# dist1ll/pomcpp

Measured on AMD Instinct MI355X. Metric: env_steps_per_sec, higher is better.
Workload: dtype int32

## Files before the change

### pomcpp_amd/csrc/pom_kernels.h

```cpp
#ifndef POM_KERNELS_H_
#define POM_KERNELS_H_

#include <hip/hip_ext.h>
#include <hip/hip_runtime.h>

#include <climits>
#include <cstdint>

#include "pom_batch.h"
#include "pom_boardgen_body.h"
#include "pom_packed.h"
#include "pom_policy_body.h"
#include "pom_step_body.h"

enum {
    ROW_BOARD = POM_REC_BOARD,
    ROW_BOMBS = POM_REC_BOMBS,
    ROW_FLAMES = POM_REC_FLAMES,
    ROW_BDEST = POM_REC_DWORDS,
    ROW_STACK = POM_REC_DWORDS + 5,
    ROW_CLAIMS = POM_REC_DWORDS + 5,
    LDS_ROWS = POM_REC_DWORDS + 36
};
static_assert(POM_REC_DWORDS % 2 == 0, "the one-lane shapes move the record in groups of 1 or 2 rows");
// ... 737 lines not shown
            const uint8_t* stage_b = reinterpret_cast<const uint8_t*>(stage);
            const int bytes = (int)(left < OBS_CODE_PASS_ENVS ? left : OBS_CODE_PASS_ENVS) * OBS_CODE_ENV_BYTES;
            uint32_t* out_w = reinterpret_cast<uint32_t*>(out_b);
#pragma unroll
            for (int i = 0; i < (OBS_CODE_PASS_ENVS * OBS_CODE_ENV_BYTES / 4 + 63) / 64; i++) {
                const int idx = lane + 64 * i;
                if (idx < (bytes >> 2)) out_w[idx] = stage_w[idx];
            }
            if (lane < (bytes & 3)) out_b[(bytes & ~3) + lane] = stage_b[(bytes & ~3) + lane];
        }
        obs_lds_order();
    }
}

template <int PE>
__device__ __forceinline__ void pom_observe_tile(const ObserveParams& p, const uint32_t* tile, uint4* stage, int64_t tile_id, int lane)
{
    static_assert(PE * POM_Q <= 64 && 16 % PE == 0, "a pass's queue slots are one round of lanes");
    if (p.dtype == POM_OBS_CODES) pom_observe_tile_codes(p, tile, stage, tile_id, lane);
    else
    for (int q = 0; q < 16 / PE; q++) {
        const int64_t e0 = tile_id * 16 + q * PE;
        if (e0 >= p.n) break;
        const int64_t left = p.n - e0;
        const int VECS = (int)(left < PE ? left : PE) * (OBS_ENV_BYTES / 16);
        constexpr int VECS_MAX = PE * OBS_ENV_BYTES / 16;
        pom_observe_stage<false, PE>(tile, stage, q, lane);
        if (p.dtype == POM_OBS_U8 && !p.per_agent) {
            uint4* out = reinterpret_cast<uint4*>(reinterpret_cast<uint8_t*>(p.planes) + e0 * OBS_ENV_BYTES);
#pragma unroll
            for (int i = 0; i < (VECS_MAX + 63) / 64; i++) {
                const int idx = lane + 64 * i;
                if (idx < VECS) out[idx] = stage[idx];
            }
        } else if (p.dtype == POM_OBS_U8) {
            obs_gather_out<uint8_t, PE>(p, reinterpret_cast<const uint32_t*>(stage), e0, lane);
        } else if (p.dtype == POM_OBS_F16) {
            obs_gather_out<_Float16, PE>(p, reinterpret_cast<const uint32_t*>(stage), e0, lane);
        } else {
            obs_gather_out<float, PE>(p, reinterpret_cast<const uint32_t*>(stage), e0, lane);
        }
        obs_lds_order();
    }
    const int ec = lane >> 2, id = lane & 3;
    const int64_t e = tile_id * 16 + ec;
    if (e < p.n && p.agent_attrs) {
        const uint32_t a0 = tile[(POM_REC_AGENTS + 2 * id) * 16 + ec], a1 = tile[(POM_REC_AGENTS + 2 * id + 1) * 16 + ec];
        const int bc = ag_bombcount((int)a0), mx = ag_max_bombs((int)a1);
        int4* o = reinterpret_cast<int4*>(p.agent_attrs + (e * 4 + id) * POM_OBS_AGENT_ATTRS);
        o[0] = make_int4(ag_x((int)a0), ag_y((int)a0), !ag_dead((int)a0), mx - bc);
        o[1] = make_int4(bc, mx, ag_strength((int)a1), ag_kick((int)a0));
    }
    if (lane < 16 && tile_id * 16 + lane < p.n && p.env_attrs) {
        const uint32_t m = pom_rec_meta(tile + lane, 16), st = (pom_rec_meta2(tile + lane, 16) >> 8) & 0xFF;
        const int status = (int)((st & POM_ST_DONE) ? 1 : 0) | (int)((st & POM_ST_DRAW) ? 2 : 0) | (int)((st & POM_ST_TIMEOUT) ? 4 : 0) |
                           (int)((st & POM_ST_RESTARTED) ? 8 : 0);
        reinterpret_cast<int4*>(p.env_attrs)[tile_id * 16 + lane] =
            make_int4((int)tile[POM_REC_TIMESTEP * 16 + lane], pom_sext8(m), status, (int)((st >> POM_ST_WINNER_SHIFT) & 7) - 1);
    }
}

#ifndef POM_QUAD_WAVES
#define POM_QUAD_WAVES 4
#endif
#ifndef POM_WPB
#define POM_WPB 1
#endif
extern "C" __device__ uint64_t pom_dispatch_id(void) __asm("llvm.amdgcn.dispatch.id");
enum { POM_CHAIN_WAIT_LIMIT_US = 2000000 };
#ifndef POM_CHAIN_WORD_STRIDE
#define POM_CHAIN_WORD_STRIDE 16
#endif

struct PomChainVisit {
    int32_t dist = 0;
    unsigned long long done = 0;
#if defined(POM_CHAIN_DIAG)
    long long t0 = 0, t1 = 0, t2 = 0, rt0 = 0;
    int polls = 0;
    uint32_t visit = 0;
#endif
};
__device__ __forceinline__ uint32_t pom_chain_xcd()
{
    uint32_t x;
    asm volatile("s_getreg_b32 %0, hwreg(HW_REG_XCC_ID)" : "=s"(x));
    return x & 0xFu;
}
__device__ __forceinline__ bool pom_chain_enter(unsigned long long* word, uint32_t chain_xcd, uint32_t chain_seq0, uint32_t tape_len, uint64_t wait_limit,
                                                uint32_t* err, int lane, PomChainVisit& v)
{
    const uint32_t xcd = chain_xcd + 1u;
#if defined(POM_CHAIN_DIAG)
    v.t0 = (long long)__builtin_readcyclecounter();
    v.rt0 = (long long)wall_clock64();
#endif
    unsigned long long w = 0;
    if (lane == 0) w = __hip_atomic_fetch_add(word, 1ull << POM_CHAIN_TICKET_SHIFT, __ATOMIC_RELAXED, __HIP_MEMORY_SCOPE_AGENT);
    w = ((unsigned long long)(uint32_t)__builtin_amdgcn_readfirstlane((int)(w >> 32)) << 32) | (uint32_t)__builtin_amdgcn_readfirstlane((int)(uint32_t)w);
    const uint32_t visit = (uint32_t)(w >> POM_CHAIN_TICKET_SHIFT);
    v.dist = (int32_t)pom_chain_visit_distance(visit, chain_seq0);
#if defined(POM_CHAIN_DIAG)
    v.t1 = (long long)__builtin_readcyclecounter();
#endif
    int polls = 0;
    bool timed_out = false;
    if (!((uint32_t)w & POM_CHAIN_POISON) && (int32_t)pom_chain_visit_distance((uint32_t)w & POM_CHAIN_COUNT_MASK, visit) < 0) {
        const uint64_t t_wait0 = wall_clock64();
        for (;;) {
            __builtin_amdgcn_s_sleep(1);
            w = __hip_atomic_load(word, __ATOMIC_RELAXED, __HIP_MEMORY_SCOPE_AGENT);
            w = ((unsigned long long)(uint32_t)__builtin_amdgcn_readfirstlane((int)(w >> 32)) << 32) | (uint32_t)__builtin_amdgcn_readfirstlane((int)(uint32_t)w);
            polls++;
            if (((uint32_t)w & POM_CHAIN_POISON) || (int32_t)pom_chain_visit_distance((uint32_t)w & POM_CHAIN_COUNT_MASK, visit) >= 0) break;
            if (wall_clock64() - t_wait0 >= wait_limit) {
                timed_out = true;
                break;
            }
        }
    }
    (void)polls;
    const uint32_t was_on = (uint32_t)(w >> 32) & 0xFu;
    const bool poisoned = ((uint32_t)w & POM_CHAIN_POISON) != 0;
    const bool wrong_xcd = was_on != 0u && was_on != xcd;
    const bool off_tape = tape_len != 0u && (uint32_t)v.dist >= tape_len;
    if (poisoned || timed_out || wrong_xcd || off_tape) {
        if (lane == 0 && !poisoned) {
            __hip_atomic_fetch_or(word, (unsigned long long)POM_CHAIN_POISON, __ATOMIC_RELAXED, __HIP_MEMORY_SCOPE_AGENT);
            __hip_atomic_fetch_or(err, (uint32_t)(timed_out ? POM_CHAIN_E_TIMEOUT : wrong_xcd ? POM_CHAIN_E_XCD : POM_CHAIN_E_TAPE), __ATOMIC_RELAXED,
                                  __HIP_MEMORY_SCOPE_AGENT);
        }
        return false;
    }
#if defined(POM_CHAIN_DIAG)
    v.t2 = (long long)__builtin_readcyclecounter();
    v.polls = polls;
    v.visit = visit;
#endif
    v.done = 1ull + ((unsigned long long)(xcd - was_on) << 32);
    return true;
}
__device__ __forceinline__ void pom_chain_leave(unsigned long long* word, int lane, const PomChainVisit& v)
{
    asm volatile("s_waitcnt vmcnt(0)" ::: "memory");
    if (lane == 0) __hip_atomic_fetch_add(word, v.done, __ATOMIC_RELAXED, __HIP_MEMORY_SCOPE_AGENT);
}

template <bool CHAIN>
__device__ __forceinline__ uint32_t pom_load_shared(const uint32_t* ptr)
{
    return CHAIN ? __hip_atomic_load(ptr, __ATOMIC_RELAXED, __HIP_MEMORY_SCOPE_AGENT) : *ptr;
}

template <int EPW, int G, bool FRESH, bool POLICY = false, bool ATEND = false, bool SINGLE = false, bool CHAIN = false, bool OBS = false>
__global__ __launch_bounds__(64 * POM_WPB, (POLICY ? 4 : G == 4 ? POM_QUAD_WAVES : EPW == 16 ? 3 : EPW == 32 ? 2 : 1)) void pom_step_kernel(StepParams p)
{
    static_assert(!CHAIN || SINGLE, "chained launches play one tick each");
    static_assert(!OBS || (SINGLE && !CHAIN && !POLICY && POM_WPB == 1), "the fused observation exists for the one-tick explicit-move shape");
    static_assert(!SINGLE || G == 4, "the one-tick instantiation exists for the quad shape");
    static_assert(G == 1 || (G == 4 && EPW == 16), "a quad per env needs 16 envs per wavefront");
    static_assert(!POLICY || G == 4, "the policy runs one agent per lane of the quad");
    static_assert(!ATEND || G == 4, "the end-of-tick reset is built for the quad shape only");
    constexpr int OBS_ROWS = (obs_stage_vecs(OBS_PASS_ENVS_FUSED) * 16 + EPW * 4 - 1) / (EPW * 4);
    constexpr int OVERLAY = POLICY ? 44 : OBS ? OBS_ROWS : 0;
    constexpr int ROWS = POM_REC_DWORDS + OVERLAY > LDS_ROWS ? POM_REC_DWORDS + OVERLAY : LDS_ROWS;
    static_assert(ROWS >= LDS_ROWS, "the tick's scratch rows fit under the overlay");
    __shared__ __attribute__((aligned(16))) uint32_t tiles_[POM_WPB][ROWS * EPW];
    uint32_t* const tile = tiles_[POM_WPB == 1 ? 0 : threadIdx.x >> 6];
    uint8_t* const danger = reinterpret_cast<uint8_t*>(tile + POM_REC_DWORDS * EPW);
    uint32_t* const sets = tile + (POM_REC_DWORDS + 32) * EPW;
    const int lane = threadIdx.x & 63;
    int64_t tile_local;
    uint32_t chain_xcd = 0;
    if (CHAIN) {
        chain_xcd = pom_chain_xcd();
        const int64_t q = gridDim.x / 8;
        int64_t k_in_xcd = (int64_t)(blockIdx.x / 8) + p.chain_rot;
        if (k_in_xcd >= q) k_in_xcd -= q;
        tile_local = (int64_t)chain_xcd * q + k_in_xcd;
        if (chain_xcd >= 8u) {
            if (lane == 0) __hip_atomic_fetch_or(p.chain_err, (uint32_t)POM_CHAIN_E_XCD, __ATOMIC_RELAXED, __HIP_MEMORY_SCOPE_AGENT);
            return;
        }
        if (POM_WPB == 1 && p.block0 + tile_local >= p.block_end) return;
    } else {
#if defined(POM_NO_XCD_REMAP)
    tile_local = blockIdx.x;
#else
    {
        const int64_t b = blockIdx.x, nb = gridDim.x, q = nb / 8, r = nb % 8, x = b % 8;
        tile_local = (x < r ? x * (q + 1) : r * (q + 1) + (x - r) * q) + b / 8;
    }
#endif
    }
    if (POM_WPB > 1) {
        tile_local = tile_local * POM_WPB + (threadIdx.x >> 6);
        if (p.block0 + tile_local >= p.block_end) return;
    }
    const int64_t tile_id = p.block0 + tile_local;
    const int64_t np = p.n_pad;
    const bool env_mode = p.mode == POM_MODE_ENV;
    const int el = lane % EPW, sub = lane / EPW;
    const int64_t e_d = tile_id * EPW + el;
    uint32_t* col_d = p.state + pom_rec_col(e_d);
    const int ec = G == 1 ? el : lane >> 2;
    const int member = G == 1 ? 0 : lane & 3;
    const int64_t e = tile_id * EPW + ec;
    const bool owner = G == 1 ? sub == 0 : member == 0;
    const bool runs = G == 1 ? sub == 0 : true;
    const bool valid = runs && e < p.n;
    const uint32_t env_key = (uint32_t)(p.env_offset + e);
    uint32_t* t = tile + ec;

#if defined(POM_DIAG)
    const long long t_begin = (long long)clock64();
#endif
    long long c_steps = 0, c_episodes = 0, c_resets = 0, c_ub = 0;

    uint32_t tick0 = CHAIN ? p.tick0 : p.tick0 + *p.tick_base;
    PomChainVisit cv;
    if (CHAIN) {
        unsigned long long* const word = p.tile_seq + tile_id * POM_CHAIN_WORD_STRIDE;
        if (!pom_chain_enter(word, chain_xcd, p.chain_seq0, p.tape_len, p.chain_wait_limit, p.chain_err, lane, cv)) return;
        tick0 += (uint32_t)cv.dist;
        load_tile16_x4<POM_REC_DWORDS, 16>(p.state + tile_id * POM_TILE_DWORDS, POM_TILE_ENVS, tile, lane);
    } else if (EPW == 16) load_tile16_x4(p.state + tile_id * POM_TILE_DWORDS, POM_TILE_ENVS, tile, lane);
    else load_tile<EPW>(col_d, POM_TILE_ENVS, tile, sub);
    uint32_t m0 = 0, m1 = 0;
    if (POLICY) {
        m0 = pom_load_shared<CHAIN>(p.agent_mem + tile_id * 64 + lane);
        m1 = pom_load_shared<CHAIN>(p.agent_mem + 4 * np + tile_id * 64 + lane);
    }
    uint64_t draw0 = 0;
    int4 moves0 = make_int4(0, 0, 0, 0);
    constexpr bool TAKES_MOVES = SINGLE || G == 1;
    if (!POLICY) {
        if (TAKES_MOVES && p.moves) {
            if (valid) moves0 = reinterpret_cast<const int4*>(p.moves)[(CHAIN ? (int64_t)cv.dist * p.n : (int64_t)0) + e];
        } else {
            if (G == 4 && !SINGLE) {
            } else if (G == 4) draw0 = pom_rng_draw_half(p.seed, env_key, tick0, member >> 1);
            else draw0 = pom_rng_draw(p.seed, env_key, tick0);
        }
    }
    asm volatile("s_waitcnt vmcnt(0)" ::: "memory");
    PomLane L;
    int time_step = 0;
    uint32_t status = 0;
    lane_from_tile(L, time_step, status, t, EPW);
    bool restarted = false;

    LdsEnv<EPW, G> acc(tile, ec, member);
    PomStepper<LdsEnv<EPW, G>> stepper(acc, L);
#if defined(POM_TRUNC)
    L.trunc = p.trunc;
#endif
#if defined(POM_DIAG)
    for (int k = 0; k < POM_PH_N; k++) L.t_acc[k] = 0;
    L.t_last = t_begin;
    POM_STAMP(L, POM_PH_LOAD);
#endif

    const int n_ticks = SINGLE ? 1 : p.ticks;
    for (int tk = 0; tk < n_ticks; tk++) {
        if (ATEND) {
        } else if (FRESH) {
            const bool reload = valid && env_mode && p.auto_reset == POM_RESET_AT_START && (status & POM_ST_DONE);
            uint64_t todo = __ballot(reload && owner);
            while (todo) {
                const int src = __builtin_amdgcn_readfirstlane(__ffsll((unsigned long long)todo) - 1);
                todo &= todo - 1;
                const int ec_u = G == 1 ? src : src >> 2;
                uint32_t ep = 0;
                if (lane == src) {
                    ep = pom_load_shared<CHAIN>(p.episode + e) + 1u;
                    p.episode[e] = ep;
                }
                ep = (uint32_t)__builtin_amdgcn_readfirstlane(__shfl((int)ep, src));
                const uint32_t key = pom_board_key(p.board_seed, (uint32_t)(p.env_offset + tile_id * EPW + ec_u), ep);
                pom_boardgen_wave<EPW, POM_REC_DWORDS>(tile, ec_u, (uint32_t)__builtin_amdgcn_readfirstlane((int)key), lane);
            }
            asm volatile("" ::: "memory");
            if (reload) lane_from_tile(L, time_step, status, t, EPW);
            restarted = reload;
            c_resets += __popcll(__ballot(reload && owner));
        } else {
            const bool reload = valid && env_mode && p.auto_reset == POM_RESET_AT_START && (status & POM_ST_DONE);
            uint64_t todo = __ballot(reload && owner);
            if (todo) {
                c_resets += __popcll(todo);
                int lane_now = lane;
                if (!SINGLE) asm volatile("" : "+v"(lane_now));
                do {
                    const int src = __builtin_amdgcn_readfirstlane(__ffsll((unsigned long long)todo) - 1);
                    todo &= todo - 1;
                    const int ec_u = G == 1 ? src : src >> 2;
                    restart_column<EPW>(tile, ec_u, p.snap + (tile_id * EPW + ec_u) * POM_REC_DWORDS, lane_now);
                } while (todo);
                asm volatile("" ::: "memory");
                if (reload) lane_from_tile(L, time_step, status, t, EPW);
            }
            restarted = reload;
        }
        const bool active = valid && !(env_mode && (status & POM_ST_DONE));
        bool newly_done = false, new_ub = false;
        int mv_own = POM_MOVE_IDLE;
        if (POLICY) {
            if (tk > 0) {
                m0 = p.agent_mem[tile_id * 64 + lane];
                m1 = p.agent_mem[4 * np + tile_id * 64 + lane];
            }
            if (restarted) m0 = m1 = 0;
            restarted = false;
            PolicyStore st{tile, t, danger + ec, sets + ec, member};
#if defined(POM_TRUNC)
            st.trunc = p.trunc;
            if (active) {
                if (p.trunc > -4) pom_policy_prepare_clear(st);
                if (p.trunc > -3) pom_policy_prepare_fill(st, PomPolicyEnv{{L.a0[0], L.a0[1], L.a0[2], L.a0[3]}, {acc.ag1(0), acc.ag1(1), acc.ag1(2), acc.ag1(3)}, L.bIdx, L.bCnt});
                if (p.trunc > -2) pom_policy_prepare_safe(st);
            }
            if (p.trunc > -1)
#else
            if (active) {
                pom_policy_prepare_clear(st);
                pom_policy_prepare_fill(st, PomPolicyEnv{{L.a0[0], L.a0[1], L.a0[2], L.a0[3]}, {acc.ag1(0), acc.ag1(1), acc.ag1(2), acc.ag1(3)}, L.bIdx, L.bCnt});
                pom_policy_prepare_safe(st);
            }
#endif
            {
                const PomPolicyEnv E{{L.a0[0], L.a0[1], L.a0[2], L.a0[3]}, {acc.ag1(0), acc.ag1(1), acc.ag1(2), acc.ag1(3)}, L.bIdx, L.bCnt};
                const uint32_t r = pom_rng_draw_half(p.seed, env_key, tick0 + (uint32_t)tk, member >> 1);
                const bool actor = active && !ag_dead(sel4(member, L.a0));
#if defined(POM_DIAG)
                long long pt_last = 0, pt_acc[POM_PP_N];
                mv_own = pom_policy_wave(st, E, member, m0, m1, actor, (int)((((r >> (16 * (member & 1))) & 0xFFFFu) * 5u) >> 16), sets, lane, pt_last, pt_acc);
#else
                mv_own = pom_policy_wave(st, E, member, m0, m1, actor, (int)((((r >> (16 * (member & 1))) & 0xFFFFu) * 5u) >> 16), sets, lane);
#endif
            }
            p.agent_mem[tile_id * 64 + lane] = m0;
            p.agent_mem[4 * np + tile_id * 64 + lane] = m1;
        }
        if (active) {
            uint32_t mvp;
            if (G == 4) {
                int mine;
                if (POLICY) {
                    mine = mv_own;
                } else if (TAKES_MOVES && p.moves) {
                    const int lo = (member & 1) ? moves0.y : moves0.x, hi = (member & 1) ? moves0.w : moves0.z;
                    mine = (member & 2) ? hi : lo;
                } else {
                    const uint32_t r = SINGLE ? (uint32_t)draw0 : pom_rng_draw_half(p.seed, env_key, tick0 + (uint32_t)tk, member >> 1);
                    mine = pom_rng_pick((r >> (16 * (member & 1))) & 0xFFFFu, p.dist);
                }
                mvp = stepper.pack_moves_quad(mine);
            } else {
                int mv[4];
                if (p.moves) {
                    mv[0] = moves0.x; mv[1] = moves0.y; mv[2] = moves0.z; mv[3] = moves0.w;
                } else {
                    const uint64_t r = tk == 0 ? draw0 : pom_rng_draw(p.seed, env_key, tick0 + (uint32_t)tk);
#pragma unroll
                    for (int i = 0; i < 4; i++) mv[i] = pom_rng_pick((uint32_t)(r >> (16 * i)) & 0xFFFFu, p.dist);
                }
                mvp = stepper.pack_moves(mv);
            }
            L.ub = 0;
            status &= ~(uint32_t)POM_ST_RESTARTED;
            POM_STAMP(L, POM_PH_RESTART);
#if defined(POM_TRUNC)
            if (p.trunc <= 0) {
            } else
#endif
            if (POLICY) {
                uint32_t* t2 = tile;
                asm volatile("" : "+v"(t2));
                LdsEnv<EPW, G> acc2(t2, ec, member);
                PomStepper<LdsEnv<EPW, G>> stepper2(acc2, L);
                stepper2.step_packed(mvp);
            } else {
                stepper.step_packed(mvp);
            }
            new_ub = L.ub != 0;
            L.ub |= (t[(POM_REC_AGENTS + 5) * EPW] >> 24) | ((t[(POM_REC_AGENTS + 7) * EPW] >> 24) << 8);
            if (env_mode) {
                time_step = (int)t[POM_REC_TIMESTEP * EPW] + 1;
                if (owner) t[POM_REC_TIMESTEP * EPW] = (uint32_t)time_step;
                status = pom_env_epilogue(L, time_step, p.max_steps, status);
                newly_done = (status & POM_ST_DONE) != 0;
            }
        }
        c_steps += __popcll(__ballot(active && owner));
        c_episodes += __popcll(__ballot(newly_done && owner));
        c_ub += __popcll(__ballot(new_ub && owner));
        if (ATEND) {
            uint64_t todo = __ballot(newly_done && owner);
            if (todo) {
                c_resets += __popcll(todo);
                if (newly_done && owner) {
#pragma unroll
                    for (int k = 0; k < 8; k++) t[(POM_REC_AGENTS + k) * EPW] = pom_lane_agent_word(L, status, k, t[(POM_REC_AGENTS + k) * EPW]);
                }
                asm volatile("" ::: "memory");
                int lane_end = lane;
                asm volatile("" : "+v"(lane_end));
                do {
                    const int src = __builtin_amdgcn_readfirstlane(__ffsll((unsigned long long)todo) - 1);
                    todo &= todo - 1;
                    const int ec_u = G == 1 ? src : src >> 2;
                    const int64_t e_u = tile_id * EPW + ec_u;
                    uint32_t* tr = p.terminal + e_u * POM_REC_DWORDS;
                    column_to_record<EPW>(tile, ec_u, tr, lane_end);
                    if (FRESH) {
                        uint32_t ep = 0;
                        if (lane == src) {
                            ep = pom_load_shared<CHAIN>(p.episode + e_u) + 1u;
                            p.episode[e_u] = ep;
                        }
                        ep = (uint32_t)__builtin_amdgcn_readfirstlane(__shfl((int)ep, src));
                        const uint32_t key = pom_board_key(p.board_seed, (uint32_t)(p.env_offset + e_u), ep);
                        pom_boardgen_wave<EPW, POM_REC_DWORDS>(tile, ec_u, (uint32_t)__builtin_amdgcn_readfirstlane((int)key), lane_end);
                    } else {
                        restart_column<EPW>(tile, ec_u, p.snap + e_u * POM_REC_DWORDS, lane_end);
                    }
                } while (todo);
                asm volatile("" ::: "memory");
                if (newly_done && runs) {
                    lane_from_tile(L, time_step, status, t, EPW);
                    status |= POM_ST_RESTARTED;
                    if (POLICY) {
                        int lane_here = lane;
                        asm volatile("" : "+v"(lane_here));
                        p.agent_mem[tile_id * 64 + lane_here] = 0u;
                        p.agent_mem[4 * np + tile_id * 64 + lane_here] = 0u;
                    }
                }
            }
        }
        POM_STAMP(L, POM_PH_EPILOGUE);
    }

    if (owner) {
#pragma unroll
        for (int k = 0; k < 8; k++) t[(POM_REC_AGENTS + k) * EPW] = pom_lane_agent_word(L, status, k, (k & 1) ? t[(POM_REC_AGENTS + k) * EPW] : 0u);
    }
    if (EPW == 16) {
        int lane_late = lane;
        asm volatile("" : "+v"(lane_late));
        store_tile16_x4<CHAIN>(p.state + tile_id * POM_TILE_DWORDS, POM_TILE_ENVS, tile, lane_late);
    } else {
        store_tile<EPW>(col_d, POM_TILE_ENVS, tile, sub, el);
    }
    if (OBS) {
        asm volatile("s_waitcnt lgkmcnt(0)" ::: "memory");
        ObserveParams op;
        op.state = nullptr;
        op.n = p.n;
        op.n_pad = p.n_pad;
        op.block0 = 0;
        op.planes = p.obs_planes;
        op.agent_attrs = p.obs_agent_attrs;
        op.env_attrs = p.obs_env_attrs;
        op.dtype = p.obs_dtype;
        op.per_agent = p.obs_per_agent;
        pom_observe_tile<OBS_PASS_ENVS_FUSED>(op, tile, reinterpret_cast<uint4*>(tile + POM_REC_DWORDS * EPW), tile_id, lane);
    }
    if (CHAIN) {
        pom_chain_leave(p.tile_seq + tile_id * POM_CHAIN_WORD_STRIDE, lane, cv);
#if defined(POM_CHAIN_DIAG)
        if (lane == 0) {
            unsigned long long* d = p.tile_seq + (p.block_end - p.block0) * POM_CHAIN_WORD_STRIDE + 68 * tile_id;
            d[4 + 2 * (cv.visit & 31)] = (unsigned long long)cv.rt0;
            d[5 + 2 * (cv.visit & 31)] = (unsigned long long)wall_clock64();
            d[0] += (unsigned long long)(cv.t1 - cv.t0);
            d[1] += (unsigned long long)(cv.t2 - cv.t1);
            d[2] += (unsigned long long)((long long)__builtin_readcyclecounter() - cv.t0);
            d[3] += (unsigned long long)cv.polls;
        }
#endif
    }

#if defined(POM_DIAG)
    asm volatile("s_waitcnt vmcnt(0)" ::: "memory");
    POM_STAMP(L, POM_PH_STORE);
    if (p.diag) {
        long long inside = 0;
        for (int k = POM_PH_X_SCAN; k <= POM_PH_X_SHORT; k++) inside += L.t_acc[k];
        long long best = inside;
        for (int o = 32; o > 0; o >>= 1) {
            const long long w = __shfl_xor(best, o);
            best = w > best ? w : best;
        }
        const uint64_t who = __ballot(inside == best);
        if (lane == __ffsll((unsigned long long)who) - 1)
            for (int k = 0; k < POM_PH_N; k++) p.diag[tile_id * POM_PH_N + k] += L.t_acc[k];
    }
#endif
    if (lane == 0) {
        unsigned long long* wc = reinterpret_cast<unsigned long long*>(p.wave_counters + tile_id * POM_CNT_N);
        __hip_atomic_fetch_add(&wc[POM_CNT_STEPS], (unsigned long long)c_steps, __ATOMIC_RELAXED, __HIP_MEMORY_SCOPE_AGENT);
        if (c_episodes) __hip_atomic_fetch_add(&wc[POM_CNT_EPISODES], (unsigned long long)c_episodes, __ATOMIC_RELAXED, __HIP_MEMORY_SCOPE_AGENT);
        if (c_resets) __hip_atomic_fetch_add(&wc[POM_CNT_RESETS], (unsigned long long)c_resets, __ATOMIC_RELAXED, __HIP_MEMORY_SCOPE_AGENT);
        if (c_ub) __hip_atomic_fetch_add(&wc[POM_CNT_UB_TICKS], (unsigned long long)c_ub, __ATOMIC_RELAXED, __HIP_MEMORY_SCOPE_AGENT);
    }
}

struct LitmusParams {
    uint32_t* data;
    unsigned long long* tile_seq;
    uint32_t* err;
    unsigned long long* out;
    int64_t tiles;
    uint32_t chain_seq0;
    uint64_t wait_limit;
};
__global__ __launch_bounds__(64) void pom_chain_litmus_kernel(LitmusParams p)
// ... 464 lines not shown
```

### pomcpp_amd/csrc/pom_step_body.h

```cpp
#ifndef POM_STEP_BODY_H_
#define POM_STEP_BODY_H_

#include "pom_packed.h"

#if defined(__clang__)
#define POM_NOUNROLL _Pragma("nounroll")
#else
#define POM_NOUNROLL
#endif
#define POM_N 11
#define POM_Q 20
#define POM_STACK_DEPTH 21

#if defined(POM_DIAG) && defined(__HIP_DEVICE_COMPILE__)
#define POM_STAMP(L, k)                                   \
    do {                                                  \
        const long long now_ = (long long)clock64();      \
        (L).t_acc[k] += now_ - (L).t_last;                \
        (L).t_last = now_;                                \
    } while (0)
#else
#define POM_STAMP(L, k) ((void)0)
#endif
#if defined(POM_TRUNC)
#define POM_CUT(L, k)                 \
    do {                              \
        if ((L).trunc <= (k)) return; \
    } while (0)
#else
#define POM_CUT(L, k) ((void)0)
#endif
enum { POM_PH_LOAD = 0, POM_PH_FLAMES, POM_PH_AGENT_PREP, POM_PH_AGENT_LOOP, POM_PH_BOMB_PASS, POM_PH_BOMB_A, POM_PH_BOMB_B,
       POM_PH_TICK_BOMBS, POM_PH_EPILOGUE, POM_PH_STORE,
       POM_PH_X_SCAN, POM_PH_X_COMMIT, POM_PH_X_EPILOGUE, POM_PH_X_NEST, POM_PH_X_SHORT, POM_PH_RESTART, POM_PH_FLAMES_DEC, POM_PH_N };

struct PomLane {
    int a0[4];
    int alive, bIdx, bCnt, fIdx, fCnt;
    uint32_t ub;
#if defined(POM_DIAG)
    long long t_last, t_acc[POM_PH_N];
#endif
#if defined(POM_TRUNC)
    int trunc;
#endif
};

POM_HD int pc_is_wood(int e) { return (unsigned)(e - POM_C_WOOD) < 5u; }
POM_HD int pc_is_powerup(int e) { return (unsigned)(e - POM_C_EXTRABOMB) < 3u; }
POM_HD int pc_is_walkable(int e) { return (int)pc_is_powerup(e) | (int)(e == 0); }
POM_HD int pc_is_flame(int e) { return e >= POM_C_FLAME; }
POM_HD int pc_is_agent(int e) { return (unsigned)(e - POM_C_AGENT) < 4u; }
POM_HD int pc_agent_id(int e) { return e - POM_C_AGENT; }
POM_HD int pc_wood_flag(int e) { return (e - POM_C_WOOD) & 3; }
POM_HD int pc_is_static_block(int e) { return (int)((unsigned)(e - POM_C_EXTRABOMB) < 8u) | (int)(e == POM_C_RIGID); }
POM_HD int pc_blocks_bomb(int e) { return (int)((unsigned)(e - POM_C_EXTRABOMB) < 12u) | (int)(e == POM_C_RIGID); }
POM_HD int pc_flag_item(int f) { return f == 0 ? 0 : f + (POM_C_EXTRABOMB - 1); }
POM_HD int pc_flame_code(int c0, int r, int i, int f) { return f == 0 ? POM_C_FLAME + c0 : POM_C_FLAGGED - 41 + 40 * f + 10 * r + i; }
POM_HD int pc_flame_pops_to(int e, int c0, int r, int i)
{
    const int k = e - (POM_C_FLAGGED - 1) - 10 * r - i;
    const int flagged = (int)(k == 0) | (int)(k == 40) | (int)(k == 80);
    const int item = POM_C_EXTRABOMB + (int)(k >= 40) + (int)(k >= 80);
    return e == POM_C_FLAME + c0 ? POM_C_PASSAGE : flagged ? item : -1;
}

POM_HD int pb_x(int b) { return b & 0xF; }
POM_HD int pb_y(int b) { return (b >> 4) & 0xF; }
POM_HD int pb_pos(int b) { return b & 0xFF; }
POM_HD int pb_id(int b) { return (b >> 8) & 0xF; }
POM_HD int pb_strength(int b) { return (b >> 12) & 0xF; }
POM_HD int pb_time(int b) { return (b >> 16) & 0xF; }
POM_HD int pb_dir(int b) { return (b >> 20) & 0xF; }
POM_HD int pb_set(int b, uint32_t mask, uint32_t v) { return (int)(((uint32_t)b & ~mask) + v); }

#if defined(__HIP_DEVICE_COMPILE__)
#define POM_IN_VGPR(x) asm("" : "+v"(x))
#else
#define POM_IN_VGPR(x) ((void)0)
#endif
POM_HD int sel4(int i, const int v[4])
{
    int v0 = v[0], v1 = v[1], v2 = v[2], v3 = v[3];
    POM_IN_VGPR(v0);
    POM_IN_VGPR(v1);
    POM_IN_VGPR(v2);
    POM_IN_VGPR(v3);
    const int lo = (i & 1) ? v1 : v0, hi = (i & 1) ? v3 : v2;
    return (i & 2) ? hi : lo;
}
POM_HD uint32_t pick4(int i, const uint32_t v[4])
{
    const uint32_t lo = (i & 1) ? v[1] : v[0], hi = (i & 1) ? v[3] : v[2];
    return (i & 2) ? hi : lo;
}
POM_HD void put4(int i, int v[4], int x)
{
    v[0] = i == 0 ? x : v[0];
    v[1] = i == 1 ? x : v[1];
    v[2] = i == 2 ? x : v[2];
    v[3] = i == 3 ? x : v[3];
}
POM_HD int ag_x(int a0) { return a0 & 0xF; }
POM_HD int ag_y(int a0) { return (a0 >> 4) & 0xF; }
POM_HD int ag_pos(int a0) { return a0 & 0xFF; }
POM_HD int ag_dead(int a0) { return (a0 >> 17) & 1; }
POM_HD int ag_kick(int a0) { return (a0 >> 16) & 1; }
POM_HD int ag_setpos(int a0, int x, int y) { return (a0 & ~0xFF) | x | (y << 4); }
POM_HD int ag_bombcount(int a0) { return pom_sext8((uint32_t)a0 >> 8); }
POM_HD int ag_bombcount_add(int a0, int d) { return (a0 & ~0xFF00) | (int)(((uint32_t)a0 + ((uint32_t)d << 8)) & 0xFF00u); }
POM_HD int ag_max_bombs(int a1) { return pom_sext16((uint32_t)a1); }
POM_HD int ag_strength(int a1) { return (a1 >> 16) & 0xFF; }
POM_HD int ag_strength_inc(int a1) { return ag_strength(a1) == 0xFF ? a1 : a1 + (1 << 16); }

POM_HD int wrap20(int p)
{
    const unsigned u = (unsigned)p, w = u - (unsigned)POM_Q;
    return (int)(u < w ? u : w);
}
POM_HD uint32_t pom_zero_bytes(uint32_t x)
{
    return ~(((x & 0x7F7F7F7Fu) + 0x7F7F7F7Fu) | x | 0x7F7F7F7Fu);
}
POM_HD int div11(int c)
{
#if defined(__HIP_DEVICE_COMPILE__)
    return __mul24(c, 373) >> 12;
#else
    return c / POM_N;
#endif
}
POM_HD int oob(int x, int y)
{
    const unsigned ux = (unsigned)x, uy = (unsigned)y;
    return (ux > uy ? ux : uy) >= (unsigned)POM_N;
}

POM_HD int mv_dx(int m) { return (int)((0x55555615u >> (2 * m)) & 3u) - 1; }
POM_HD int mv_dy(int m) { return (int)((0x55555561u >> (2 * m)) & 3u) - 1; }

template <class A>
struct PomStepper {
    A& a;
    PomLane& L;
    uint32_t oldp_ = 0;
    int irregular_ = 0;
    int folded_ = 0;
    uint32_t occ_[4] = {0u, 0u, 0u, 0u};
    int occ_valid_ = 0, occ_keep_ = 0;
    POM_HD PomStepper(A& a_, PomLane& l_) : a(a_), L(l_) {}

    POM_HD int bomb_at(int i) const { return a.bomb(wrap20(L.bIdx + i)); }
    POM_HD void set_bomb_at(int i, int v) { a.set_bomb(wrap20(L.bIdx + i), v); }

    POM_HD int bomb_index(int pos) const
    {
        int r = 99;
        POM_NOUNROLL
        for (int i = a.sub(); i < L.bCnt; i += A::G) {
            if (pb_pos(bomb_at(i)) == pos) {
                r = i;
                break;
            }
        }
        r = a.gmin(r);
        return r == 99 ? -1 : r;
    }
    POM_HD void put_bomb_at(int i, int v) { a.put_bomb(wrap20(L.bIdx + i), v); }
    POM_HD int bomb_index_alone(int pos) const
    {
        POM_NOUNROLL
        for (int i = 0; i < L.bCnt; i += 4) {
            const int b0 = bomb_at(i), b1 = bomb_at(i + 1), b2 = bomb_at(i + 2), b3 = bomb_at(i + 3);
            int r = -1;
            r = ((int)(i + 3 < L.bCnt) & (int)(pb_pos(b3) == pos)) ? i + 3 : r;
            r = ((int)(i + 2 < L.bCnt) & (int)(pb_pos(b2) == pos)) ? i + 2 : r;
            r = ((int)(i + 1 < L.bCnt) & (int)(pb_pos(b1) == pos)) ? i + 1 : r;
            r = pb_pos(b0) == pos ? i : r;
            if (r >= 0) return r;
        }
        return -1;
    }

    POM_HD int get_agent(int x, int y) const
    {
        const int want = x | (y << 4);
        int r = -1;
#pragma unroll
        for (int i = 3; i >= 0; i--)
            r = ((!ag_dead(L.a0[i])) & (int)(ag_pos(L.a0[i]) == want)) ? i : r;
        return r;
    }

    POM_HD void kill(int id)
    {
        if (id >= POM_AGENT_COUNT) {
            L.ub |= POM_UB_BAD_INDEX;
            return;
        }
        int v = sel4(id, L.a0);
        if (!ag_dead(v)) {
            put4(id, L.a0, v | POM_AG_DEAD);
            L.alive--;
        }
    }

    POM_HD void owner_bombcount_dec(int b)
    {
        int id = pb_id(b);
        if (id >= POM_AGENT_COUNT) {
            L.ub |= POM_UB_BAD_INDEX;
            return;
        }
        put4(id, L.a0, ag_bombcount_add(sel4(id, L.a0), -1));
    }

    POM_HD void remove_at(int at)
    {
        POM_NOUNROLL
        for (int i = at + 1 + a.sub(); i < L.bCnt; i += A::G) {
            const int v = bomb_at(i);
            put_bomb_at(i - 1, v);
        }
        a.sync();
        if (folded_) {
            const int w = bomb_at(L.bCnt - 1);
            set_bomb_at(L.bCnt - 1, (w & (1 << 24)) ? (w & ~(1 << 24)) : (int)((uint32_t)w + (1u << 16)));
        }
        L.bCnt--;
    }

    enum { REM_TOP = 62, REM_NONE = 63 };

    POM_HD int owner_strength(int b)
    {
        const int owner = pb_id(b);
        if (owner < POM_AGENT_COUNT) return ag_strength(a.ag1(owner));
        L.ub |= POM_UB_BAD_INDEX;
        return 0;
    }
// ... 469 lines not shown
                POM_NOUNROLL
                for (int i = a.sub(); i < L.bCnt; i += A::G) {
                    if (a.bdest(i) == okey) {
                        bd = i;
                        break;
                    }
                }
                bd = a.gmin(bd);
                if (bd == 99) bd = -1;
            }
            put4(id, L.a0, ag_setpos(av, ox, oy));
            irregular_ |= (ox | (oy << 4)) != (int)((oldp_ >> (8 * id)) & 0xFF);
            a.set_cell(oy * POM_N + ox, POM_C_AGENT + id);
            if (origin_agent != -1) {
                id = origin_agent;
                continue;
            }
            if (bd != -1) {
                const int b = bomb_at(bd);
                const int dir = pb_dir(b);
                if (mv_dx(dir) == 0 && mv_dy(dir) == 0) {
                    a.set_cell(oy * POM_N + ox, POM_C_AGENT + id);
                    return;
                }
                const int bx = ox - mv_dx(dir), by = oy - mv_dy(dir);
                if (oob(bx, by)) {
                    L.ub |= POM_UB_BAD_INDEX;
                    return;
                }
                const int has_agent = get_agent(bx, by);
                set_bomb_at(bd, pb_set(pb_set(b, 0xF00000u, 0), 0xFFu, (uint32_t)bx + ((uint32_t)by << 4)));
                a.set_cell(by * POM_N + bx, POM_C_BOMB);
                if (has_agent != -1) {
                    id = has_agent;
                    continue;
                }
            }
            return;
        }
    }

    POM_HD int bomb_target_key(int b) const
    {
        const int d = pb_dir(b);
        return (pb_x(b) + mv_dx(d) + 1) | ((pb_y(b) + mv_dy(d) + 1) << 4);
    }

    POM_HD int bomb_collision(uint32_t mvp, int k)
    {
        const int b = bomb_at(k);
        const int key = bomb_target_key(b);
        int collided = 0;
        POM_NOUNROLL
        for (int i = k + a.sub(); i < L.bCnt; i += A::G) {
            const int o = bomb_at(i);
            if (o != b && bomb_target_key(o) == key) {
                put_bomb_at(i, pb_set(o, 0xF00000u, 0));
                collided = 1;
            }
        }
        collided = a.gor(collided);
        if (collided && pb_dir(b) != 0) {
            const int nb = pb_set(b, 0xF00000u, 0);
            set_bomb_at(k, nb);
            const int ag = get_agent(pb_x(nb), pb_y(nb));
            if (ag > -1) {
                const int m = (mvp >> (4 * ag)) & 0xF;
                if (m != POM_MOVE_IDLE && m != POM_MOVE_BOMB) {
                    unforeseen_ = 1;
                    chain_reversion(mvp, ag);
                    const int cur = bomb_at(k);
                    a.set_cell(pb_y(cur) * POM_N + pb_x(cur), POM_C_BOMB);
                }
            }
        }
        return collided;
    }

    POM_HD void loop_a_bomb(int mvp, int oldp, int k, int bombs_move)
    {
        const int b = bomb_at(k);
        const int bx = pb_x(b), by = pb_y(b), d = pb_dir(b);
        const int tx = bx + mv_dx(d), ty = by + mv_dy(d);
        int blocked = oob(tx, ty);
        if (!blocked) {
            const int e = a.cell(ty * POM_N + tx);
            blocked = pc_blocks_bomb(e);
        }
        if (blocked) {
            set_bomb_at(k, pb_set(b, 0xF00000u, 0));
            const int ag = get_agent(bx, by);
            if (ag > -1) {
                const int m = (mvp >> (4 * ag)) & 0xF;
                const int av = sel4(ag, L.a0);
                const int was = (oldp >> (8 * ag)) & 0xFF;
                if ((int)(m != POM_MOVE_IDLE) & (int)(m != POM_MOVE_BOMB) & (int)((ag_x(av) | (ag_y(av) << 4)) != was)) {
                    chain_reversion(mvp, ag, bombs_move);
                    if (get_agent(bx, by) == -1) a.set_cell(by * POM_N + bx, POM_C_BOMB);
                }
            }
        }
    }

    POM_HD void step(const int mv_in[4]) { step_packed(pack_moves(mv_in)); }
    POM_HD static int clamp_move(int m) { return ((unsigned)m <= 5u) ? m : 6; }
    POM_HD static uint32_t pack_moves(const int mv_in[4])
    {
        uint32_t mvp = 0;
#pragma unroll
        for (int i = 0; i < 4; i++) mvp |= (uint32_t)clamp_move(mv_in[i]) << (4 * i);
        return mvp;
    }
    POM_HD uint32_t pack_moves_quad(int mine) const
    {
        const int c = clamp_move(mine);
        return (uint32_t)a.template gbcast<0>(c) | ((uint32_t)a.template gbcast<1>(c) << 4) | ((uint32_t)a.template gbcast<2>(c) << 8) |
               ((uint32_t)a.template gbcast<3>(c) << 12);
    }
    POM_HD void step_packed(uint32_t mvp)
    {
        int ftop, fn, btop, bn;
        flames_dec(ftop, fn);
        POM_STAMP(L, POM_PH_FLAMES_DEC);
        POM_CUT(L, 10);
        flame_pops(ftop, fn);
        POM_STAMP(L, POM_PH_FLAMES);
        POM_CUT(L, 20);
        step_middle(mvp, btop, bn);
        top_explosions(btop, bn);
        POM_STAMP(L, POM_PH_TICK_BOMBS);
    }
    POM_HD void top_explosions(int top, int n)
    {
        occ_valid_ = 0;
        occ_keep_ = 1;
        POM_NOUNROLL
        for (int k = 0; k < n && L.bCnt > 0; k++) {
            const int c = k == 0 ? top : bomb_at(0);
            if (pb_time(c) != 0) break;
            explode(pb_x(c), pb_y(c), pb_strength(c), REM_TOP, c);
        }
        occ_valid_ = occ_keep_ = 0;
    }
    POM_HD void prep_positions(const uint32_t mvp, uint32_t& oldp, uint32_t& dstp, int& deadmask, int& contact, int& clash)
    {
        oldp = dstp = 0;
        deadmask = 0;
#pragma unroll
        for (int i = 0; i < 4; i++) deadmask |= ag_dead(L.a0[i]) << i;
        contact = 0;
        clash = 0;
        if (A::G == 4) {
            const int m = a.sub();
            const int av = sel4(m, L.a0);
            const int mvm = (int)((mvp >> (4 * m)) & 0xF);
            const int pxm = ag_x(av), pym = ag_y(av);
            const int dxm = pxm + mv_dx(mvm), dym = pym + mv_dy(mvm);
            const int pos8 = ag_pos(av);
            oldp = (uint32_t)a.template gbcast<0>(pos8) | ((uint32_t)a.template gbcast<1>(pos8) << 8) |
                   ((uint32_t)a.template gbcast<2>(pos8) << 16) | ((uint32_t)a.template gbcast<3>(pos8) << 24);
            const int d8 = ((dxm + 1) & 0xF) | (((dym + 1) & 0xF) << 4);
            dstp = (uint32_t)a.template gbcast<0>(d8) | ((uint32_t)a.template gbcast<1>(d8) << 8) |
                   ((uint32_t)a.template gbcast<2>(d8) << 16) | ((uint32_t)a.template gbcast<3>(d8) << 24);
            const uint32_t want = (uint32_t)((dxm & 0xF) | ((dym & 0xF) << 4));
            const uint32_t others = ~(0x80u << (8 * m));
            const uint32_t dead80 = (((uint32_t)deadmask * 0x00204081u) & 0x01010101u) << 7;
            const uint32_t hit_d = pom_zero_bytes(oldp ^ (want * 0x01010101u)) & others;
            const uint32_t hit_p = pom_zero_bytes(oldp ^ ((uint32_t)pos8 * 0x01010101u)) & others & ~dead80;
            int mine = (int)(hit_d != 0u) | ((int)((hit_p != 0u) & !ag_dead(av)) << 1);
            mine = a.gor(mine);
            contact = mine & 1;
            clash = mine >> 1;
        } else {
#pragma unroll
            for (int i = 0; i < 4; i++) {
                const int px = ag_x(L.a0[i]), py = ag_y(L.a0[i]);
                const int mvi = (int)((mvp >> (4 * i)) & 0xF);
                const int dx = px + mv_dx(mvi), dy = py + mv_dy(mvi);
                oldp |= (uint32_t)(px | (py << 4)) << (8 * i);
                dstp |= (uint32_t)(((dx + 1) & 0xF) | (((dy + 1) & 0xF) << 4)) << (8 * i);
            }
#pragma unroll
            for (int i = 0; i < 4; i++)
#pragma unroll
                for (int j = 0; j < 4; j++)
                    if (i != j) contact |= ((((dstp >> (8 * i)) & 0xF) - 1) & 0xF) == ((oldp >> (8 * j)) & 0xF) &&
                                           ((((dstp >> (8 * i + 4)) & 0xF) - 1) & 0xF) == ((oldp >> (8 * j + 4)) & 0xF);
        }
    }
    POM_HD void prep_dependencies(const uint32_t mvp, const uint32_t oldp, const int deadmask, uint32_t& dstp, uint32_t& dep, uint32_t& roots,
                                  int& nroots)
    {
        int px[4], py[4], dx[4], dy[4];
#pragma unroll
        for (int i = 0; i < 4; i++) {
            px[i] = (int)((oldp >> (8 * i)) & 0xF);
            py[i] = (int)((oldp >> (8 * i + 4)) & 0xF);
            const int mvi = (int)((mvp >> (4 * i)) & 0xF);
            dx[i] = px[i] + mv_dx(mvi);
            dy[i] = py[i] + mv_dy(mvi);
        }
        roots = 0xFFFF;
        nroots = 0;
#pragma unroll
        for (int i = 0; i < 4; i++) {
#pragma unroll
            for (int j = i; j < 4; j++) {
                if ((int)(dx[i] == px[j]) & (int)(dy[i] == py[j]) & (int)(dx[j] == px[i]) & (int)(dy[j] == py[i])) {
                    dx[i] = px[i]; dy[i] = py[i];
                    dx[j] = px[j]; dy[j] = py[j];
                }
            }
        }
#pragma unroll
        for (int i = 0; i < 4; i++) {
            int is_root = 1;
            if (!((deadmask >> i) & 1)) {
#pragma unroll
                for (int j = 0; j < 4; j++) {
                    if (j == i) continue;
                    if (is_root & !((deadmask >> j) & 1) & (int)(dx[i] == px[j]) & (int)(dy[i] == py[j])) {
                        dep = (dep & ~(0xFu << (4 * j))) | ((uint32_t)i << (4 * j));
                        is_root = 0;
                    }
                }
            }
            if (is_root) {
                roots = (roots & ~(0xFu << (4 * nroots))) | ((uint32_t)i << (4 * nroots));
                nroots++;
            }
        }
        dstp = 0;
#pragma unroll
        for (int i = 0; i < 4; i++) dstp |= (uint32_t)(((dx[i] + 1) & 0xF) | (((dy[i] + 1) & 0xF) << 4)) << (8 * i);
    }

    int unforeseen_ = 0;
    POM_HD uint32_t loop_b_todo()
    {
        a.claims_clear();
        a.sync();
        POM_NOUNROLL
        for (int k = a.sub(); k < L.bCnt; k += A::G) {
            const int b = bomb_at(k);
            const int d = pb_dir(b);
            const int bx = pb_x(b), by = pb_y(b), tx = bx + mv_dx(d), ty = by + mv_dy(d);
            a.claim(by * POM_N + bx);
            if ((int)(d != 0) & !oob(tx, ty) & (int)((mv_dx(d) | mv_dy(d)) != 0)) a.claim(ty * POM_N + tx);
        }
        a.sync();
        uint32_t f = 0;
        POM_NOUNROLL
        for (int k = a.sub(); k < L.bCnt; k += A::G) {
            const int b = bomb_at(k);
            const int c = pb_y(b) * POM_N + pb_x(b);
            const int e = a.cell(c);
            f |= (uint32_t)((int)(pb_dir(b) != 0) | (int)(e == POM_C_PASSAGE) | pc_is_flame(e) | (int)(a.claims(c) >= 2)) << k;
        }
        return (uint32_t)a.gor((int)f);
    }
    POM_HD void loop_b_bomb(uint32_t mvp, int k)
    {
        int b = bomb_at(k);
        const int bx = pb_x(b), by = pb_y(b), d = pb_dir(b);
        int tx = bx, ty = by;
        if (d == 0) {
            if (bomb_collision(mvp, k)) return;
            const int c = by * POM_N + bx;
            const int e = a.cell(c);
            if (e == POM_C_PASSAGE) a.set_cell(c, POM_C_BOMB);
            if (!pc_is_flame(e)) return;
        } else {
            tx = bx + mv_dx(d);
            ty = by + mv_dy(d);
            int free_way = !oob(tx, ty);
            int tc = 0, te = 0;
            if (free_way) {
                tc = ty * POM_N + tx;
                te = a.cell(tc);
                free_way = !pc_is_static_block(te);
            }
            if (!free_way) {
                set_bomb_at(k, pb_set(b, 0xF00000u, 0));
                return;
            }
            if (bomb_collision(mvp, k)) return;
            b = bomb_at(k);
            set_bomb_at(k, pb_set(b, 0xFFu, (uint32_t)tx + ((uint32_t)ty << 4)));
            if (bomb_index(bx | (by << 4)) < 0 && a.cell(by * POM_N + bx) == POM_C_BOMB)
                a.set_cell(by * POM_N + bx, POM_C_PASSAGE);
            te = a.cell(tc);
            if (pc_is_walkable(te)) a.set_cell(tc, POM_C_BOMB);
            if (!pc_is_flame(te)) return;
        }
        const int j = bomb_index(tx | (ty << 4));
        const int jb = bomb_at(j);
        unforeseen_ = 1;
        explode(pb_x(jb), pb_y(jb), owner_strength(jb), j);
    }

    POM_HD void step_middle(const uint32_t mvp, int& top, int& n)
    {
        top = 0;
        n = 0;

        uint32_t oldp = 0, dstp = 0;
        uint32_t dep = 0xFFFF, roots = 0x3210;
        int nroots = 4;
        int deadmask = 0, contact = 0, clash = 0;
        prep_positions(mvp, oldp, dstp, deadmask, contact, clash);
        oldp_ = oldp;
        POM_CUT(L, 24);
        if (contact) prep_dependencies(mvp, oldp, deadmask, dstp, dep, roots, nroots);
        POM_CUT(L, 27);
        const int ouroboros = nroots == 0;
        int posb[4];
#pragma unroll
        for (int i = 0; i < 4; i++) posb[i] = (int)((oldp >> (8 * i)) & 0xFF);

        int on_bomb = 0;
        POM_NOUNROLL
        for (int k = a.sub(); k < L.bCnt; k += A::G) {
// ... 385 lines not shown
```

Measured before the change: 8.936 billion.

## Build quad old positions locally, drop VGPR pins, specialise uniform move pick

In the quad prep path, the packed old-position word is now built directly from the agent records each lane already holds, instead of four cross-lane broadcasts. The own agent's position and dead flag are then taken from that word and the dead mask. The VGPR-pinning asm is removed from sel4. Random move picking goes through a helper that does a plain multiply-shift for the non-stress distributions, with empty asm barriers added around the branches. Together these aim to cut cross-lane traffic and selection overhead, but the asm barriers may also constrain scheduling.

```diff
diff --git a/pomcpp_amd/csrc/pom_kernels.h b/pomcpp_amd/csrc/pom_kernels.h
--- a/pomcpp_amd/csrc/pom_kernels.h
+++ b/pomcpp_amd/csrc/pom_kernels.h
@@ -913,6 +913,19 @@
     return CHAIN ? __hip_atomic_load(ptr, __ATOMIC_RELAXED, __HIP_MEMORY_SCOPE_AGENT) : *ptr;
 }
 
+__device__ __forceinline__ int pom_pick_uniform(uint32_t r16, int dist)
+{
+    int mv;
+    if (dist == POM_DIST_STRESS) {
+        asm volatile("");
+        mv = pom_rng_pick(r16, POM_DIST_STRESS);
+    } else {
+        asm volatile("");
+        mv = (int)((r16 * (dist == POM_DIST_HARMLESS ? 5u : 6u)) >> 16);
+    }
+    return mv;
+}
+
 template <int EPW, int G, bool FRESH, bool POLICY = false, bool ATEND = false, bool SINGLE = false, bool CHAIN = false, bool OBS = false>
 __global__ __launch_bounds__(64 * POM_WPB, (POLICY ? 4 : G == 4 ? POM_QUAD_WAVES : EPW == 16 ? 3 : EPW == 32 ? 2 : 1)) void pom_step_kernel(StepParams p)
 {
@@ -1110,11 +1123,13 @@
                 if (POLICY) {
                     mine = mv_own;
                 } else if (TAKES_MOVES && p.moves) {
+                    asm volatile("");
                     const int lo = (member & 1) ? moves0.y : moves0.x, hi = (member & 1) ? moves0.w : moves0.z;
                     mine = (member & 2) ? hi : lo;
                 } else {
+                    asm volatile("");
                     const uint32_t r = SINGLE ? (uint32_t)draw0 : pom_rng_draw_half(p.seed, env_key, tick0 + (uint32_t)tk, member >> 1);
-                    mine = pom_rng_pick((r >> (16 * (member & 1))) & 0xFFFFu, p.dist);
+                    mine = pom_pick_uniform((r >> (16 * (member & 1))) & 0xFFFFu, p.dist);
                 }
                 mvp = stepper.pack_moves_quad(mine);
             } else {
@@ -1124,7 +1139,7 @@
                 } else {
                     const uint64_t r = tk == 0 ? draw0 : pom_rng_draw(p.seed, env_key, tick0 + (uint32_t)tk);
 #pragma unroll
-                    for (int i = 0; i < 4; i++) mv[i] = pom_rng_pick((uint32_t)(r >> (16 * i)) & 0xFFFFu, p.dist);
+                    for (int i = 0; i < 4; i++) mv[i] = pom_pick_uniform((uint32_t)(r >> (16 * i)) & 0xFFFFu, p.dist);
                 }
                 mvp = stepper.pack_moves(mv);
             }
diff --git a/pomcpp_amd/csrc/pom_step_body.h b/pomcpp_amd/csrc/pom_step_body.h
--- a/pomcpp_amd/csrc/pom_step_body.h
+++ b/pomcpp_amd/csrc/pom_step_body.h
@@ -81,11 +81,7 @@
 #endif
 POM_HD int sel4(int i, const int v[4])
 {
-    int v0 = v[0], v1 = v[1], v2 = v[2], v3 = v[3];
-    POM_IN_VGPR(v0);
-    POM_IN_VGPR(v1);
-    POM_IN_VGPR(v2);
-    POM_IN_VGPR(v3);
+    const int v0 = v[0], v1 = v[1], v2 = v[2], v3 = v[3];
     const int lo = (i & 1) ? v1 : v0, hi = (i & 1) ? v3 : v2;
     return (i & 2) ? hi : lo;
 }
@@ -861,13 +857,12 @@
         clash = 0;
         if (A::G == 4) {
             const int m = a.sub();
-            const int av = sel4(m, L.a0);
+#pragma unroll
+            for (int i = 0; i < 4; i++) oldp |= (uint32_t)ag_pos(L.a0[i]) << (8 * i);
+            const int pos8 = (int)((oldp >> (8 * m)) & 0xFF);
             const int mvm = (int)((mvp >> (4 * m)) & 0xF);
-            const int pxm = ag_x(av), pym = ag_y(av);
+            const int pxm = pos8 & 0xF, pym = pos8 >> 4;
             const int dxm = pxm + mv_dx(mvm), dym = pym + mv_dy(mvm);
-            const int pos8 = ag_pos(av);
-            oldp = (uint32_t)a.template gbcast<0>(pos8) | ((uint32_t)a.template gbcast<1>(pos8) << 8) |
-                   ((uint32_t)a.template gbcast<2>(pos8) << 16) | ((uint32_t)a.template gbcast<3>(pos8) << 24);
             const int d8 = ((dxm + 1) & 0xF) | (((dym + 1) & 0xF) << 4);
             dstp = (uint32_t)a.template gbcast<0>(d8) | ((uint32_t)a.template gbcast<1>(d8) << 8) |
                    ((uint32_t)a.template gbcast<2>(d8) << 16) | ((uint32_t)a.template gbcast<3>(d8) << 24);
@@ -876,7 +871,7 @@
             const uint32_t dead80 = (((uint32_t)deadmask * 0x00204081u) & 0x01010101u) << 7;
             const uint32_t hit_d = pom_zero_bytes(oldp ^ (want * 0x01010101u)) & others;
             const uint32_t hit_p = pom_zero_bytes(oldp ^ ((uint32_t)pos8 * 0x01010101u)) & others & ~dead80;
-            int mine = (int)(hit_d != 0u) | ((int)((hit_p != 0u) & !ag_dead(av)) << 1);
+            int mine = (int)(hit_d != 0u) | ((int)((hit_p != 0u) & !((deadmask >> m) & 1)) << 1);
             mine = a.gor(mine);
             contact = mine & 1;
             clash = mine >> 1;
```

Result: no change. 8.968 billion (median of 3 runs) (+0.4%).
